# artis-mcrt/artis

Measured on AMD Instinct MI355X. Metric: packet-steps/sec, higher is better.
Workload: dtype f64

## Files before the change

artis_amd/csrc/artis_engine.hip:

```cpp
#include <hip/hip_runtime.h>
#include <rccl/rccl.h>

#include <dlfcn.h>

#include <cstdio>
#include <cstdlib>
#include <algorithm>
#include <chrono>
#include <cstring>
#include <string>
#include <type_traits>
#include <utility>
#include <vector>
#include <cmath>

#include "model_build.h"
#include "engine_config.h"
#include "cache_residency.h"
#include "physics.h"
#include "radfield_fit.h"
#include "ion_balance.h"
#include "decay_update.h"
#include "deposition.h"
#include "spectra.h"
// ... 1050 lines not shown
        Q.s0[s] = w.s0; Q.s1[s] = w.s1; Q.s2[s] = w.s2; Q.s3[s] = w.s3;
        Q.lv[s] = w.ma_level | (k.start << 16);
        Q.cnt[s] = units | (k.njumps << 16);
        Q.ready[nready + __popcll(pm & (lanebit - 1ull))] = (uint8_t)s;
      }
      nready += __popcll(pm);
#ifdef ARTIS_PROFILE
      if (lane == 0) {
        ARTIS_STAT_ADD(env, 46, prof_rounds);
        ARTIS_STAT_ADD(env, 45, prof_lanes);
      }
#endif
      __builtin_amdgcn_wave_barrier();
      TQ_PROF(43);
    }
  }
  __syncthreads();
  if (threadIdx.x < ARTIS_NSTATS && lstats[threadIdx.x] != 0) atomicAdd(&gstats[threadIdx.x], lstats[threadIdx.x]);
}
#ifndef ARTIS_TQ_TB
#define ARTIS_TQ_TB 768
#endif
constexpr int TQ_TB = ARTIS_TQ_TB;
inline size_t tq_lds_bytes(int tb, int nlevels, int nalltrans) {
  return (((sizeof(TQWave) * (size_t)(tb / 64)) + 15) & ~(size_t)15) + (sizeof(LevelPack) * (size_t)nlevels) + (sizeof(uint32_t) * (size_t)((nalltrans + 1) / 2));
}

#ifndef ARTIS_LATE_KERNEL
#define ARTIS_LATE_KERNEL (!ARTIS_OPT_VPKT_ON && !ARTIS_OPT_DETAILED_BF_ESTIMATORS_ON)
#endif
#ifndef ARTIS_LATE_TB
#define ARTIS_LATE_TB 512
#endif
constexpr int LATE_TB = ARTIS_LATE_TB;
constexpr size_t LATE_LDS_HEAD = (sizeof(stat_t) * ARTIS_NSTATS) + 64;
inline size_t late_lds_bytes(int nlevels, int nalltrans, int nbfcontinua) {
  return LATE_LDS_HEAD + (sizeof(LevelPack) * (size_t)nlevels) + (((sizeof(uint32_t) * (size_t)((nalltrans + 1) / 2)) + 15) & ~(size_t)15) +
         (sizeof(ContPack) * (size_t)nbfcontinua);
}
struct LateArgs {
  const int32_t *list[2];
  int32_t n[2];
  int32_t *ring[2];
  int32_t *bailouts;
  int32_t poll_cap;
};
#if ARTIS_LATE_KERNEL
struct LateRing {
  int32_t *ring;
  uint32_t cap;
  int32_t *head, *res, *pub;
};
__device__ inline void late_push(const LateRing &Q, bool flag, int32_t pi, int32_t *errflag) {
  const unsigned long long mask = __ballot(flag);
  if (mask == 0) return;
  const int lane = threadIdx.x & 63;
  const int cnt = __popcll(mask);
  const int prefix = __popcll(mask & ((1ull << lane) - 1ull));
  const int leader = __ffsll((long long)mask) - 1;
  int base = 0;
  if (lane == leader) base = atomicAdd(Q.res, cnt);
  base = __shfl(base, leader);
  if (flag) Q.ring[(uint32_t)(base + prefix) % Q.cap] = pi;
  __builtin_amdgcn_fence(__ATOMIC_RELEASE, "workgroup");
  if (lane == leader) {
    int spins = 0;
    bool turn = true;
    while (__hip_atomic_load(Q.pub, __ATOMIC_RELAXED, __HIP_MEMORY_SCOPE_WORKGROUP) != base) {
      __builtin_amdgcn_s_sleep(1);
      if (++spins > (1 << 24)) {
        if (errflag) *errflag = 47;
        turn = false;
        break;
      }
    }
    if (turn) __hip_atomic_store(Q.pub, base + cnt, __ATOMIC_RELEASE, __HIP_MEMORY_SCOPE_WORKGROUP);
  }
}
__device__ inline int32_t late_pull(const LateRing &Q, bool need) {
  const unsigned long long mask = __ballot(need);
  if (mask == 0) return -1;
  const int lane = threadIdx.x & 63;
  const int prefix = __popcll(mask & ((1ull << lane) - 1ull));
  const int leader = __ffsll((long long)mask) - 1;
  int h = 0, t = 0;
  if (lane == leader) {
    h = __hip_atomic_load(Q.head, __ATOMIC_RELAXED, __HIP_MEMORY_SCOPE_WORKGROUP);
    t = __hip_atomic_load(Q.pub, __ATOMIC_ACQUIRE, __HIP_MEMORY_SCOPE_WORKGROUP);
  }
  h = __shfl(h, leader);
  t = __shfl(t, leader);
  const int take = min(__popcll(mask), t - h);
  if (take <= 0) return -1;
  int32_t v = -1;
  if (need && prefix < take) v = __hip_atomic_load(&Q.ring[(uint32_t)(h + prefix) % Q.cap], __ATOMIC_RELAXED, __HIP_MEMORY_SCOPE_WORKGROUP);
  int ok = 0;
  if (lane == leader) ok = (atomicCAS(Q.head, h, h + take) == h) ? 1 : 0;
  ok = __shfl(ok, leader);
  __builtin_amdgcn_fence(__ATOMIC_ACQUIRE, "workgroup");
  return ok ? v : -1;
}
struct LateSink {
  LateRing q[2];
  int32_t *live;
  int32_t *errflag;
  __device__ void put(bool left, int kind, int32_t pi, const Pkt &p, const Lists &next) const {
    const bool to_r = left && kind == NEXT_RPKT;
    const bool to_t = left && (kind == NEXT_MA || kind == NEXT_KPKT);
    late_push(q[0], to_r, pi, errflag);
    late_push(q[1], to_t, pi, errflag);
    const bool out = left && !to_r && !to_t;
    append_by_kind(out ? kind : NEXT_DONE, pi, p.cellindex, p.nu_cmf, next, (p.ma_element * 5 + p.ma_ion));
    const unsigned long long om = __ballot(out);
    if (om != 0 && (int)(threadIdx.x & 63) == __ffsll((long long)om) - 1) atomicSub(live, __popcll(om));
  }
};
__global__ void __launch_bounds__(LATE_TB, 1) k_late(Env env, LateArgs a, Lists next, unsigned long long *gstats) {
  extern __shared__ __attribute__((aligned(16))) unsigned char late_lds[];
  const int64_t nwg = gridDim.x, b = xcd_chunk(blockIdx.x, nwg);
  const int32_t r0 = (int32_t)(((int64_t)a.n[0] * b) / nwg), r1 = (int32_t)(((int64_t)a.n[0] * (b + 1)) / nwg);
  const int32_t t0 = (int32_t)(((int64_t)a.n[1] * b) / nwg), t1 = (int32_t)(((int64_t)a.n[1] * (b + 1)) / nwg);
  const int32_t own = (r1 - r0) + (t1 - t0);
  if (own == 0) return;
  stat_t *lstats = (stat_t *)late_lds;
  int32_t *ctr = (int32_t *)(late_lds + (sizeof(stat_t) * ARTIS_NSTATS));
  LevelPack *lds_levelpack = (LevelPack *)(late_lds + LATE_LDS_HEAD);
  uint16_t *lds_tlevel = (uint16_t *)(lds_levelpack + env.M.nlevels);
  ContPack *lds_cont = (ContPack *)((unsigned char *)lds_tlevel + (((sizeof(uint32_t) * (size_t)((env.M.nalltrans + 1) / 2)) + 15) & ~(size_t)15));
  if (threadIdx.x < ARTIS_NSTATS) lstats[threadIdx.x] = 0;
  for (int i = threadIdx.x; i < env.M.nlevels; i += LATE_TB) lds_levelpack[i] = env.M.level_pack[i];
  {
    const uint32_t *src = (const uint32_t *)env.M.alltrans_tlevel16;
    uint32_t *dst = (uint32_t *)lds_tlevel;
    for (int i = threadIdx.x; i < (env.M.nalltrans + 1) / 2; i += LATE_TB) dst[i] = src[i];
  }
  {
    const D2 *src = (const D2 *)env.M.cont_pack;
    D2 *dst = (D2 *)lds_cont;
    for (int i = threadIdx.x; i < env.M.nbfcontinua * 2; i += LATE_TB) dst[i] = src[i];
  }
  LateSink sink{{{a.ring[0] + (r0 + t0), (uint32_t)own, ctr + 0, ctr + 2, ctr + 4}, {a.ring[1] + (r0 + t0), (uint32_t)own, ctr + 1, ctr + 3, ctr + 5}},
                ctr + 6, env.errflag};
  for (int i = threadIdx.x; i < r1 - r0; i += LATE_TB) sink.q[0].ring[i] = a.list[0][r0 + i];
  for (int i = threadIdx.x; i < t1 - t0; i += LATE_TB) sink.q[1].ring[i] = a.list[1][t0 + i];
  if (threadIdx.x == 0) {
    ctr[0] = ctr[1] = 0;
    ctr[2] = ctr[4] = r1 - r0;
    ctr[3] = ctr[5] = t1 - t0;
    ctr[6] = own;
  }
  env.M.level_pack = lds_levelpack;
  env.M.alltrans_tlevel16 = lds_tlevel;
  env.ma_tables_in_lds = 1;
  env.M.cont_pack = lds_cont;
  env.cont_in_lds = 1;
  env.cellest_lds = nullptr;
  env.cellest_n = 0;
  env.estcache = nullptr;
  env.estcache_nv = 0;
  __syncthreads();
  env.stats = lstats;
  const double ts_end = env.S.ts_end;
  constexpr int NW = LATE_TB / 64;
  int nw_r = (int)((((int64_t)(r1 - r0) * NW) + (own / 2)) / own);
  if (r1 > r0 && t1 > t0) nw_r = max(1, min(NW - 1, nw_r));
  int role = __builtin_amdgcn_readfirstlane(((int)(threadIdx.x >> 6) < nw_r) ? 0 : 1);
  bool have = false;
  int32_t pi = 0;
  int n_it = 0;
  int polls = 0;
  Pkt p;
  Chi x;
  MACtx k;
  long long tprev = 0;
  while (true) {
    const int32_t got = late_pull(sink.q[role], !have);
    if (got >= 0) {
      pi = got;
      if (role == 0) {
        pkt_load(env.P, pi, p);
        chi_load(env.P, pi, p, x);
      } else {
        pkt_load_thermal(env.P, pi, p);
        k = ma_ctx(env, p);
      }
      have = true;
    }
    if (!__any(have)) {
      const int mine = __hip_atomic_load(ctr + 4 + role, __ATOMIC_RELAXED, __HIP_MEMORY_SCOPE_WORKGROUP) -
                       __hip_atomic_load(ctr + role, __ATOMIC_RELAXED, __HIP_MEMORY_SCOPE_WORKGROUP);
      const int other = __hip_atomic_load(ctr + 5 - role, __ATOMIC_RELAXED, __HIP_MEMORY_SCOPE_WORKGROUP) -
                        __hip_atomic_load(ctr + 1 - role, __ATOMIC_RELAXED, __HIP_MEMORY_SCOPE_WORKGROUP);
      if (__builtin_amdgcn_readfirstlane(mine) > 0) continue;
      if (__builtin_amdgcn_readfirstlane(other) > 0) {
        role = 1 - role;
        continue;
      }
      if (__builtin_amdgcn_readfirstlane(__hip_atomic_load(ctr + 6, __ATOMIC_RELAXED, __HIP_MEMORY_SCOPE_WORKGROUP)) == 0) break;
      if (++polls > a.poll_cap) {
        if ((threadIdx.x & 63) == 0) atomicAdd(a.bailouts, 1);
        break;
      }
      __builtin_amdgcn_s_sleep(64);
      continue;
    }
    polls = 0;
    const bool held = have;
    constexpr bool COLD = false;
#define ROUND_LEAVE(n) false
#define ROUND_BEFORE_LEAVE
#define ROUND_PUT(kind_, pi_) sink.put(held && !have, kind_, pi_, p, next)
    if (role == 0) {
      int &steps = n_it;
#include "rpkt_round.inc"
    } else {
      int &units = n_it;
#include "thermal_round.inc"
    }
#undef ROUND_LEAVE
#undef ROUND_BEFORE_LEAVE
#undef ROUND_PUT
  }
  __syncthreads();
  if (threadIdx.x < ARTIS_NSTATS && lstats[threadIdx.x] != 0) atomicAdd(&gstats[threadIdx.x], lstats[threadIdx.x]);
}
#endif

struct TailLists {
  const int32_t *list[4];
// ... 286 lines not shown
        continue;
      }
      if (have) have = vray_step(env, ray);
    }
  } else {
    for (int64_t i = (int64_t)blockIdx.x * TB + threadIdx.x; i < n64; i += (int64_t)gridDim.x * TB) {
      const VpktSeed seed = queue[i / nobs];
      vpkt_trace_seed_direction(env, seed, (int)(i % nobs));
    }
  }
  __syncthreads();
  if (threadIdx.x < ARTIS_NSTATS && lstats[threadIdx.x] != 0) atomicAdd(&gstats[threadIdx.x], lstats[threadIdx.x]);
}
#endif

inline int nblocks(int64_t n) { return (int)((n + BLOCK - 1) / BLOCK); }

struct SpecState;
void spec_free(SpecState *st);
struct RfState;
void rf_free(RfState *st);
struct IbState;
void ib_free(IbState *st);
struct DecayState;
void decay_free(DecayState *st);
struct DepState;
void dep_free(DepState *st);

}

struct LastCall {
  double propagate_ms = 0., kms[NEXT_NKINDS] = {}, kms_tail = 0., fill_ms = 0.;
  double kms_late = 0.;
  int64_t late_launches = 0;
  int64_t late_bailouts = 0;
  int64_t klaunches[NEXT_NKINDS] = {}, kthreads[NEXT_NKINDS] = {}, nlaunches = 0;
  int64_t sweeps = 0, tile_fills = 0, sparse_fills = 0, cells_filled = 0, listed = 0, parked = 0;
  int64_t pool_resets = 0;
  int32_t thermal_variants = 0, est_forms = 0;
};
struct SortScratch {
  void *base = nullptr;
  int64_t capacity = 0;
  int2 *pairs = nullptr;
  int32_t *mat = nullptr;
  int32_t *tiles = nullptr;
  int32_t *seg = nullptr;
  int32_t *chunk_base = nullptr;
};
struct CellCache {
  int ntiles = 1;
  int tile_lo = 0, tile_hi = 0;
  int tile_valid_lo = -1;
  artis_residency::Residency res;
  int32_t *d_krow = nullptr;
  std::vector<int32_t> h_cell_grid;
  size_t cache_bytes_per_cell = 0;
  int32_t *d_fill_cells = nullptr;
  bool sparse_fill = true;
  int64_t sparse_max_listed = 16384;
  bool tile_adapt = true;
  int64_t tile_block = 0;
  bool pool_keep = true;
  int32_t *d_waiting = nullptr;
  std::vector<int32_t> h_waiting;
  double *d_collexc_terms = nullptr;
  int64_t pop_batch = 0;
// ... 43 lines not shown
  int64_t npackets = -1;
  void *d_pkt = nullptr;
  void *d_pkt_snapshot = nullptr;
  size_t pkt_bytes = 0;
  PktStore P{};
  artis_packet *d_aos = nullptr;
  int64_t aos_capacity = 0;
  bool aos_valid = false;
  int32_t *d_lists[NEXT_NKINDS][2] = {};
  int32_t *d_keys[NEXT_NKINDS][2] = {};
  int32_t *d_sorted = nullptr;
  int32_t *d_perm = nullptr;
  bool use_perm = false;
  bool slot_order_by_cell = true;
  int32_t *d_hist = nullptr;
  int32_t *d_tiles = nullptr;
  SortScratch sort_scratch;
  bool sort_attr_set = false;
  int32_t *d_count = nullptr;
  int32_t *d_cursors = nullptr;
  int ncu = 256;
  double *d_gamma_ws = nullptr;
  int32_t *d_gamma_gi = nullptr;
  int32_t *d_gamma_n = nullptr;
  int64_t ws_capacity = 0;
  hipEvent_t ev0 = nullptr, ev1 = nullptr, ev2 = nullptr, ev3 = nullptr;
  LastCall last;
  int tail_max = ARTIS_OPT_DETAILED_BF_ESTIMATORS_ON ? 16384 : 4096;
  bool tail_always = false;
  int64_t late_max = 200000;
  bool late_always = false;
  bool late_strict = false;
  bool late_attr_set = false;
  int32_t *d_late_ring[2] = {nullptr, nullptr};
  int32_t *d_late_bail = nullptr;
  bool park_tails = true;
  int64_t park_at = 3145728;
  int64_t last_pool_used = 0, last_pool_cap = 0;
  double ma_hotfrac = 1.;
  bool vpkt_cont_lds = true;
  bool tile_zigzag = false;
  int64_t last_visits = 0;
  int budget_r = (ARTIS_OPT_RPKT_BB_THERMALISATION || ARTIS_OPT_VPKT_ON) ? 8 : 4;
  int budget_g = ARTIS_OPT_DETAILED_BF_ESTIMATORS_ON ? 32 : 64;
  int budget_t = ARTIS_OPT_DETAILED_BF_ESTIMATORS_ON ? 1024 : 2048;
  int small_list = 300000;
  int budget_t_small = 0;
  int budget_r_small = 0;
  int drain_t = 48;
  int drain_r = 1;
  int64_t drain_min_list = 1000000;
  bool sort_lists = true;
  bool sort_nu = true;
  bool sort_numajor = true;
  int sort_cellshift = 0;
  bool sort_ma = true;
  bool rpkt_est_over_cont = true;
  int ma_bins = SORT_MABINS;
  bool ma_filters = true;
  int dense_lpr = 32;
  bool dense_cont_lds = true;
  bool cellest_in_lds = true;
  bool estcache = true;
  int sort_maxpc_r = 20000;
  int sort_maxpc_t = 600;
  bool wave_chunks_r = true, wave_chunks_t = false;
  bool cu_chunks_t = false;
  bool cont_lds = true;
// ... 192 lines not shown
  const int32_t matlen = nb * ntiles;
  const int nscan = (matlen + SCAN_TILE - 1) / SCAN_TILE;
  const size_t lds = sizeof(int32_t) * 2 * ((size_t)1 << lobits);
  if (lds > 32 * 1024 && !e->sort_attr_set) {
    HIP_TRY(hipFuncSetAttribute((const void *)k_sort_segments, hipFuncAttributeMaxDynamicSharedMemorySize, (int)(sizeof(int32_t) * 2 << SORT_LO_BITS_MAX)));
    e->sort_attr_set = true;
  }
  hipLaunchKernelGGL(k_sort_tilehist, dim3(ntiles), dim3(SORT_TB), 0, s, keys, n, lobits, nb, ntiles, S.mat);
  hipLaunchKernelGGL(k_scan_tiles, dim3(nscan), dim3(1024), 0, s, S.mat, matlen, S.tiles);
  if (nscan > 1) {
    hipLaunchKernelGGL(k_scan_totals, dim3(1), dim3(1024), 0, s, S.tiles, nscan);
    hipLaunchKernelGGL(k_scan_add, dim3(nscan), dim3(1024), 0, s, S.mat, matlen, S.tiles);
  }
  hipLaunchKernelGGL(k_sort_tilescatter, dim3(ntiles), dim3(SORT_TB), 0, s, list, keys, n, lobits, nb, ntiles, S.mat, S.pairs);
  hipLaunchKernelGGL(k_sort_plan, dim3(1), dim3(1024), 0, s, S.mat, ntiles, nb, n, S.seg, S.chunk_base);
  hipLaunchKernelGGL(k_sort_segments, dim3(n / SORT_SEG_CAP + nb), dim3(BLOCK), lds, s, S.pairs, lobits, nb, S.seg, S.chunk_base, out);
  return ARTIS_OK;
}
int sort_list(artis_amd_engine *e, hipStream_t s, const int32_t *list, const int32_t *keys, int32_t n, int64_t nkeys, int32_t *out) {
  if (nkeys > SORT_LDS_KEYS) return sort_many_keys(e, e->sort_scratch, s, list, keys, n, nkeys, out);
  const int32_t nk = (int32_t)nkeys;
  HIP_TRY(hipMemsetAsync(e->d_hist, 0, sizeof(int32_t) * (size_t)(nk + 1), s));
  hipLaunchKernelGGL(k_sort_hist_lds, dim3(sort_lds_grid(n)), dim3(BLOCK), 0, s, keys, n, e->d_hist, nk);
  const int ntiles = (nk + SCAN_TILE - 1) / SCAN_TILE;
  hipLaunchKernelGGL(k_scan_tiles, dim3(ntiles), dim3(1024), 0, s, e->d_hist, nk, e->d_tiles);
  hipLaunchKernelGGL(k_scan_totals, dim3(1), dim3(1024), 0, s, e->d_tiles, ntiles);
  hipLaunchKernelGGL(k_scan_add, dim3(ntiles), dim3(1024), 0, s, e->d_hist, nk, e->d_tiles);
  hipLaunchKernelGGL(k_sort_scatter_lds, dim3(sort_lds_grid(n)), dim3(BLOCK), 0, s, list, keys, n, e->d_hist, out, nk);
  return ARTIS_OK;
}

void free_packet_buffers(artis_amd_engine *e) {
  void **singles[] = {&e->d_pkt, &e->d_pkt_snapshot, (void **)&e->d_sorted, (void **)&e->d_perm, (void **)&e->d_gamma_ws,
                      (void **)&e->d_late_ring[0], (void **)&e->d_late_ring[1],
                      (void **)&e->d_gamma_gi, (void **)&e->d_gamma_n, (void **)&e->d_bfev, (void **)&e->d_bfev_count,
                      (void **)&e->d_vpkt_queue, (void **)&e->d_vpkt_count};
  e->bfev_cap = 0;
  e->vpkt_cap = 0;
  sort_scratch_free(e->sort_scratch);
  for (void **q : singles) {
    if (*q) (void)hipFree(*q);
    *q = nullptr;
  }
  for (int kind = 0; kind < NEXT_NKINDS; kind++)
    for (int k = 0; k < 2; k++) {
      if (e->d_lists[kind][k]) (void)hipFree(e->d_lists[kind][k]);
      if (e->d_keys[kind][k]) (void)hipFree(e->d_keys[kind][k]);
      e->d_lists[kind][k] = nullptr;
      e->d_keys[kind][k] = nullptr;
    }
  e->npackets = -1;
  e->use_perm = false;
}

bool late_possible(const artis_amd_engine *e) {
  return ARTIS_LATE_KERNEL && e->late_max > 0 && e->tail_max > 0 && e->cc.ntiles == 1 && e->Mh.ncold == 0 && e->Mh.nlevels > 0 && e->Mh.nlevels < 32768 &&
         e->Mh.nalltrans > 0 && e->Mh.nbfcontinua > 0 && late_lds_bytes(e->Mh.nlevels, e->Mh.nalltrans, e->Mh.nbfcontinua) <= 160 * 1024 - 1024;
}
int ensure_packet_buffers(artis_amd_engine *e, int64_t n) {
  if (n == e->npackets && e->d_pkt) return ARTIS_OK;
  free_packet_buffers(e);
  e->pkt_bytes = pkt_store_bytes(n);
  HIP_TRY(hipMalloc(&e->d_pkt, e->pkt_bytes));
  e->P = carve_pkt_store(e->d_pkt, n);
  const size_t listbytes = sizeof(int32_t) * (size_t)(n > 0 ? n : 1);
  for (int kind = 1; kind < NEXT_NKINDS; kind++)
    for (int k = 0; k < 2; k++) {
      HIP_TRY(hipMalloc((void **)&e->d_lists[kind][k], listbytes));
      HIP_TRY(hipMalloc((void **)&e->d_keys[kind][k], listbytes));
    }
  HIP_TRY(hipMalloc((void **)&e->d_sorted, listbytes));
  HIP_TRY(hipMalloc((void **)&e->d_perm, listbytes));
  if (late_possible(e)) {
    for (int k = 0; k < 2; k++) HIP_TRY(hipMalloc((void **)&e->d_late_ring[k], listbytes));
  }
  if (const int rc = sort_scratch_alloc(e->sort_scratch, n)) return rc;
  e->ws_capacity = n > 0 ? n : 1;
  const size_t wsbytes = sizeof(double) * (size_t)(e->Mh.nbfcontinua_ground + 1) * (size_t)e->ws_capacity;
  HIP_TRY(hipMalloc((void **)&e->d_gamma_ws, wsbytes));
  HIP_TRY(hipMalloc((void **)&e->d_gamma_gi, wsbytes / 2));
  HIP_TRY(hipMalloc((void **)&e->d_gamma_n, sizeof(int32_t) * (size_t)e->ws_capacity));
  HIP_TRY(hipMemset(e->d_gamma_n, 0, sizeof(int32_t) * (size_t)e->ws_capacity));
#if ARTIS_OPT_DETAILED_BF_ESTIMATORS_ON
  if (e->Mh.nbfcontinua > 0) {
    const int64_t cap = std::min<int64_t>((int64_t)(n > 0 ? n : 1) * e->budget_r, 0x7FFFFFF0LL);
    HIP_TRY(hipMalloc((void **)&e->d_bfev, sizeof(BfEvent) * (size_t)cap));
    HIP_TRY(hipMalloc((void **)&e->d_bfev_count, sizeof(int32_t)));
    HIP_TRY(hipMemset(e->d_bfev_count, 0, sizeof(int32_t)));
    e->bfev_cap = (int32_t)cap;
  }
#endif
#if ARTIS_OPT_VPKT_ON
  {
    const int64_t cap = std::min<int64_t>((int64_t)(n > 0 ? n : 1) * std::max(e->budget_r, 1), 0x7FFFFFF0LL);
    HIP_TRY(hipMalloc((void **)&e->d_vpkt_queue, sizeof(VpktSeed) * (size_t)cap));
    HIP_TRY(hipMalloc((void **)&e->d_vpkt_count, sizeof(int32_t)));
    HIP_TRY(hipMemset(e->d_vpkt_count, 0, sizeof(int32_t)));
    e->vpkt_cap = (int32_t)cap;
  }
#endif
  e->npackets = n;
  return ARTIS_OK;
}

int ensure_aos(artis_amd_engine *e, int64_t n) {
  if (n <= e->aos_capacity && e->d_aos) return ARTIS_OK;
  if (e->d_aos) (void)hipFree(e->d_aos);
// ... 1032 lines not shown
  if (!e) return ARTIS_ERR_ARG;
  if (sweeps) *sweeps = e->last.sweeps;
  if (tile_fills) *tile_fills = e->last.tile_fills;
  if (fill_ms) *fill_ms = e->last.fill_ms;
  if (listed) *listed = e->last.listed;
  return ARTIS_OK;
}

int artis_amd_last_kernel_table(artis_amd_engine *e, double ms[4], int64_t launches[4], int64_t packets[4]) {
  if (!e) return ARTIS_ERR_ARG;
  const int kinds[4] = {NEXT_RPKT, NEXT_MA, NEXT_KPKT, NEXT_SLOW};
  for (int i = 0; i < 4; i++) {
    if (ms) ms[i] = e->last.kms[kinds[i]];
    if (launches) launches[i] = e->last.klaunches[kinds[i]];
    if (packets) packets[i] = e->last.kthreads[kinds[i]];
  }
  return ARTIS_OK;
}

int artis_amd_last_kernel_ms_by_kind(artis_amd_engine *e, double ms[8], int64_t launches[8]) {
  if (!e || !ms) return ARTIS_ERR_ARG;
  const int kinds[5] = {NEXT_RPKT, NEXT_MA, NEXT_SLOW, NEXT_GAMMA, NEXT_BB};
  for (int i = 0; i < 8; i++) {
    ms[i] = 0.;
    if (launches) launches[i] = 0;
  }
  for (int i = 0; i < 5; i++) {
    ms[i] = e->last.kms[kinds[i]];
    if (launches) launches[i] = e->last.klaunches[kinds[i]];
  }
  ms[5] = e->last.kms_tail;
  ms[6] = e->last.fill_ms;
  ms[7] = e->last.kms_late;
  if (launches) launches[7] = e->last.late_launches;
  return ARTIS_OK;
}

int artis_amd_debug_visit_counts(artis_amd_engine *e, uint32_t *counts, int64_t n) {
  if (!e || !counts || n != (int64_t)e->Mh.npts_nonempty * e->Mh.nlevels) {
    g_last_error = "visit counts: [npts_nonempty][nlevels] uint32 expected";
    return ARTIS_ERR_ARG;
  }
  if (e->d_visit_counts == nullptr) {
    g_last_error = "this library was not built with -DARTIS_VISIT_COUNTS (or no propagation call has run yet)";
    return ARTIS_ERR_ARG;
  }
  HIP_TRY(hipSetDevice(e->device));
  HIP_TRY(hipMemcpy(counts, e->d_visit_counts, sizeof(uint32_t) * (size_t)n, hipMemcpyDeviceToHost));
  return ARTIS_OK;
}

int artis_amd_debug_sort_list(artis_amd_engine *e, const int32_t *keys, const int32_t *list, int32_t n, int64_t nkeys, int32_t *out) {
  if (!e || n < 0 || (n > 0 && (!keys || !list || !out))) {
    g_last_error = "null argument or negative length";
    return ARTIS_ERR_ARG;
  }
  if (nkeys <= SORT_LDS_KEYS) {
    g_last_error = "debug_sort_list runs the many-keys sort: nkeys has to be above " + std::to_string(SORT_LDS_KEYS);
    return ARTIS_ERR_ARG;
  }
  if (nkeys > SORT_MAX_KEYS) {
    g_last_error = sort_too_many_keys_text(nkeys);
    return ARTIS_ERR_UNSUPPORTED;
  }
  for (int32_t i = 0; i < n; i++)
    if (keys[i] < 0 || keys[i] >= nkeys) {
      g_last_error = "a key is outside [0, nkeys)";
// ... 43 lines not shown
```

artis_amd/csrc/stage_propagate.h:

```cpp
#pragma once
namespace {
#define STEP(expr)                     \
  do {                                 \
    const int _rc = (expr);            \
    if (_rc != ARTIS_OK) return _rc;   \
  } while (0)
template <int N>
using Int = std::integral_constant<int, N>;
int sort_by_key(artis_amd_engine *e, hipStream_t s, const int32_t *list, const int32_t *keys, int32_t n, const int32_t **out, int nbins,
                int64_t ncells, int max_per_cell, int32_t nkeys_given = 0, int32_t *into = nullptr) {
  *out = list;
  if (!e->sort_lists || n < 2 * BLOCK) return ARTIS_OK;
  if ((int64_t)n > (int64_t)max_per_cell * (ncells > 0 ? ncells : 1)) return ARTIS_OK;
  if (into == nullptr) into = e->d_sorted;
  STEP(sort_list(e, s, list, keys, n, nkeys_given > 0 ? (int64_t)nkeys_given : (int64_t)e->Mh.ngrid * nbins, into));
  *out = into;
  return ARTIS_OK;
}
#if ARTIS_OPT_DETAILED_BF_ESTIMATORS_ON
void launch_bfest_dense(artis_amd_engine *e, const Env &env, hipStream_t s) {
  const bool lds = e->dense_cont_lds && e->Mh.nbfcontinua <= CONT_LDS_MAX;
  e->last.est_forms |= (lds ? ARTIS_AMD_EST_BF_DENSE_CONTLDS : ARTIS_AMD_EST_BF_DENSE_HBM) |
                       (e->dense_lpr == 64 ? ARTIS_AMD_EST_BF_LPR64 : (e->dense_lpr == 16 ? ARTIS_AMD_EST_BF_LPR16 : ARTIS_AMD_EST_BF_LPR32));
  auto launch = [&](auto lpr) {
// ... 208 lines not shown
      e->last.thermal_variants |= ARTIS_AMD_THERMAL_PLAIN;
      e->last.est_forms |= thermal_est_form(env, 0);
      launch(Int<ARTIS_THERMAL_TB>{}, Int<0>{}, grid, per_cu ? 256 : chunk_count(e->wave_chunks_t, nk, grid * (ARTIS_THERMAL_TB / 64)), per_cu ? 2 : 0);
    }
    return ARTIS_OK;
  }
  void launch_gamma(const int32_t *lst, int32_t nk, const Lists &next) {
    const int grid = std::min(nblocks(nk), e->ncu * ARTIS_GAMMA_WAVES);
    e->last.est_forms |= env.cellest_n_g > 0 ? ARTIS_AMD_EST_GAMMA_LDS : ARTIS_AMD_EST_GAMMA_GLOBAL;
    hipLaunchKernelGGL(k_gamma, dim3(grid), dim3(BLOCK), 0, s, env, lst, nk, next, e->d_stats, e->budget_g, e->d_cursors,
                       chunk_count(e->wave_chunks_r, nk, grid * (BLOCK / 64)));
  }
  int launch_vpkt_followup([[maybe_unused]] int kind) {
#if ARTIS_OPT_VPKT_ON
    if (kind != NEXT_GAMMA && kind != NEXT_BB) {
      HIP_TRY(hipMemsetAsync(e->d_cursors, 0, sizeof(int32_t) * (MAX_CHUNKS + 1), s));
      if (e->vpkt_cont_lds && e->Mh.nbfcontinua <= CONT_LDS_MAX && e->Mh.nbfcontinua > 0)
        hipLaunchKernelGGL((k_vpkt<true, ARTIS_VPKT_TB>), dim3(e->ncu), dim3(ARTIS_VPKT_TB), 0, s, env, e->d_stats, e->d_cursors);
      else
        hipLaunchKernelGGL((k_vpkt<false, BLOCK>), dim3(e->ncu * ARTIS_VPKT_WGS), dim3(BLOCK), 0, s, env, e->d_stats, e->d_cursors);
      HIP_TRY(hipMemsetAsync(e->d_vpkt_count, 0, sizeof(int32_t), s));
    }
#endif
    return ARTIS_OK;
  }
  int finish_launch(int kind, bool tail, int32_t n) {
    HIP_TRY(hipEventRecord(e->ev1, s));
    if (!tail) wall_launch += since(t_launch);
    STEP(read_counts());
    float ms = 0.f;
    HIP_TRY(hipEventElapsedTime(&ms, e->ev0, e->ev1));
    e->last.nlaunches++;
    (tail ? e->last.kms_tail : e->last.kms[kind]) += ms;
    if (!tail) {
      e->last.klaunches[kind]++;
      e->last.kthreads[kind] += n;
      visit_launches++;
    }
    if (e->trace && tail)
      fprintf(stderr, "[artis_amd] launch %lld tail n=%d+0 %.3f ms -> r %d ma %d slow %d gamma %d bb %d\n", (long long)e->last.nlaunches, n, ms, cnt[NEXT_RPKT], cnt[NEXT_MA], cnt[NEXT_NKINDS], cnt[NEXT_GAMMA], cnt[NEXT_BB]);
    else if (e->trace)
      fprintf(stderr, "[artis_amd] launch %lld kind %d n=%d %.3f ms -> r %d ma %d slow %d k %d self %d\n", (long long)e->last.nlaunches, kind, n, ms, cnt[NEXT_RPKT], cnt[NEXT_MA], cnt[NEXT_SLOW], cnt[NEXT_KPKT], cnt[NEXT_NKINDS]);
    cur[kind] = 1 - cur[kind];
    cnt[kind] = cnt[NEXT_NKINDS];
    HIP_TRY(hipMemcpyAsync(e->d_count + kind, e->d_count + NEXT_NKINDS, sizeof(int32_t), hipMemcpyDeviceToDevice, s));
    if (++guard > 2000000LL) {
      g_last_error = "packet loop did not terminate";
      return ARTIS_ERR_NOTCONVERGED;
    }
    return ARTIS_OK;
  }
  static constexpr int tail_kinds[4] = {NEXT_RPKT, NEXT_MA, NEXT_SLOW, NEXT_BB};
  int64_t count_tail() const { return (int64_t)cnt[NEXT_RPKT] + cnt[NEXT_MA] + cnt[NEXT_SLOW] + cnt[NEXT_BB]; }
  int run_tail(int64_t tail_n) {
    TailLists in;
    for (int i = 0; i < 4; i++) {
      in.list[i] = e->d_lists[tail_kinds[i]][cur[tail_kinds[i]]];
      in.n[i] = cnt[tail_kinds[i]];
      HIP_TRY(hipMemsetAsync(e->d_count + tail_kinds[i], 0, sizeof(int32_t), s));
    }
    HIP_TRY(hipMemsetAsync(e->d_count + NEXT_NKINDS, 0, sizeof(int32_t), s));
    STEP(reset_pool_if_due());
    HIP_TRY(hipEventRecord(e->ev0, s));
    e->last.thermal_variants |= ARTIS_AMD_THERMAL_TAIL;
    hipLaunchKernelGGL(k_tail, dim3(nblocks(tail_n * 64)), dim3(BLOCK), 0, s, env, in, lists_for(NEXT_SLOW), e->d_stats);
    STEP(flush_bf_events());
    return finish_launch(NEXT_SLOW, true, (int32_t)tail_n);
  }
  int sort_current(int kind, const int32_t **lst, int32_t *into = nullptr) {
    *lst = e->d_lists[kind][cur[kind]];
    if (kind == NEXT_RPKT || kind == NEXT_GAMMA || (kind == NEXT_MA && e->sort_ma)) {
      STEP(sort_by_key(e, s, e->d_lists[kind][cur[kind]], e->d_keys[kind][cur[kind]], cnt[kind], lst,
                       kind == NEXT_RPKT ? r_nubins : (kind == NEXT_MA ? e->ma_bins : 1), e->cc.res.tile_cells,
                       kind == NEXT_MA ? (env.cellest_n_t > 0 ? INT32_MAX : e->sort_maxpc_t) : (env.cellest_n_r > 0 ? INT32_MAX : e->sort_maxpc_r),
                       (kind == NEXT_RPKT && r_nubins > 1 && e->sort_numajor) ? r_ngroups * r_nubins : 0, into));
    }
    return ARTIS_OK;
  }
  bool late_eligible() const { return late_possible(e) && e->d_late_ring[0] != nullptr; }
  int run_late() {
#if ARTIS_LATE_KERNEL
    LateArgs a;
    const int kinds[2] = {NEXT_RPKT, NEXT_MA};
    const clk::time_point t_sort = clk::now();
    for (int i = 0; i < 2; i++) {
      STEP(sort_current(kinds[i], &a.list[i], e->d_lists[kinds[i]][1 - cur[kinds[i]]]));
      a.n[i] = cnt[kinds[i]];
      a.ring[i] = e->d_late_ring[i];
    }
    wall_sort += since(t_sort);
    a.bailouts = e->d_late_bail;
    a.poll_cap = 1 << 20;
    const size_t lds = late_lds_bytes(e->Mh.nlevels, e->Mh.nalltrans, e->Mh.nbfcontinua);
    if (!e->late_attr_set) {
      HIP_TRY(hipFuncSetAttribute((const void *)k_late, hipFuncAttributeMaxDynamicSharedMemorySize, 160 * 1024 - 1024));
      e->late_attr_set = true;
    }
    for (int i = 0; i < 2; i++) HIP_TRY(hipMemsetAsync(e->d_count + kinds[i], 0, sizeof(int32_t), s));
    HIP_TRY(hipMemsetAsync(e->d_late_bail, 0, sizeof(int32_t), s));
    HIP_TRY(hipEventRecord(e->ev0, s));
    e->last.thermal_variants |= ARTIS_AMD_THERMAL_LATE;
    hipLaunchKernelGGL(k_late, dim3(e->ncu), dim3(LATE_TB), lds, s, env, a, lists_for(0), e->d_stats);
    HIP_TRY(hipEventRecord(e->ev1, s));
    STEP(read_counts());
    const int32_t bail = e->h_counts[(2 * NEXT_NKINDS) + 1];
    float ms = 0.f;
    HIP_TRY(hipEventElapsedTime(&ms, e->ev0, e->ev1));
    e->last.nlaunches++;
    e->last.kms_late += ms;
    e->last.late_launches++;
    e->last.late_bailouts += bail;
    if (e->trace)
      fprintf(stderr, "[artis_amd] launch %lld late n=%d+%d %.3f ms -> slow %d gamma %d bb %d; %d waves gave up waiting\n", (long long)e->last.nlaunches, a.n[0],
              a.n[1], ms, cnt[NEXT_SLOW], cnt[NEXT_GAMMA], cnt[NEXT_BB], bail);
    if (bail != 0 && e->late_strict) {
      g_last_error = "k_late: " + std::to_string(bail) + " waves gave up waiting for work (ARTIS_AMD_LATE_STRICT=1)";
      return ARTIS_ERR_NOTCONVERGED;
    }
    if (++guard > 2000000LL) {
      g_last_error = "packet loop did not terminate";
      return ARTIS_ERR_NOTCONVERGED;
    }
#endif
    return ARTIS_OK;
  }
  int run_kind(int kind) {
    const int32_t nk = cnt[kind];
    const Lists next = lists_for(kind);
    const int32_t *lst = e->d_lists[kind][cur[kind]];
    const clk::time_point t_sort = clk::now();
    STEP(sort_current(kind, &lst));
    wall_sort += since(t_sort);
    t_launch = clk::now();
    if (kind == NEXT_SLOW) STEP(reset_pool_if_due());
    hipLaunchKernelGGL(k_launch_reset, dim3(1), dim3(BLOCK), 0, s, e->d_count, kind, e->d_cursors);
    HIP_TRY(hipEventRecord(e->ev0, s));
    if (kind == NEXT_RPKT)
      STEP(launch_rpkt(lst, nk, next));
    else if (kind == NEXT_GAMMA)
      launch_gamma(lst, nk, next);
    else if (kind == NEXT_MA)
      STEP(launch_thermal(lst, nk, next));
    else if (kind == NEXT_BB)
      hipLaunchKernelGGL(k_blackbody, dim3(nblocks(nk)), dim3(BLOCK), 0, s, env, lst, nk, next, e->d_stats);
    else
      hipLaunchKernelGGL(k_slow, dim3(nblocks(nk)), dim3(BLOCK), 0, s, env, lst, nk, next, e->d_stats);
    STEP(launch_vpkt_followup(kind));
    return finish_launch(kind, false, nk);
  }
  bool should_park(int sweep, int tile, int64_t tail_n, bool tail_now) {
    if (!e->park_tails || e->cc.ntiles <= 1 || visit_launches == 0) return false;
    if (e->park_at > e->tail_max && listed > e->park_at && tail_n > 0 && tail_n + cnt[NEXT_KPKT] <= e->park_at) {
      e->last.parked += tail_n + cnt[NEXT_KPKT] + cnt[NEXT_GAMMA];
      if (e->trace) fprintf(stderr, "[artis_amd] sweep %d tile %d: %lld packets parked (park_at)\n", sweep, tile, (long long)(tail_n + cnt[NEXT_KPKT]));
      return true;
    }
    if (tail_now && listed > e->tail_max) {
      e->last.parked += tail_n + cnt[NEXT_GAMMA];
      if (e->trace) fprintf(stderr, "[artis_amd] sweep %d tile %d: %lld packets parked\n", sweep, tile, (long long)tail_n);
      return true;
    }
    return false;
  }
  int run_visit(int sweep, int tile) {
    static constexpr int order[6] = {NEXT_SLOW, NEXT_GAMMA, NEXT_BB, NEXT_KPKT, NEXT_MA, NEXT_RPKT};
    e->last_visits++;
    listed = count_listed();
    e->last.listed += listed;
    visit_launches = 0;
    if (e->trace) fprintf(stderr, "[artis_amd] sweep %d tile %d of %d\n", sweep, tile, e->cc.ntiles);
    const bool tail_ok = e->tail_max > 0 && (e->tail_always || listed > e->tail_max || sweep > 0 || (adaptive && e->last_visits > e->cc.ntiles));
    const bool late_ok = late_eligible() && (e->late_always || listed > e->late_max);
    while (count_listed() > 0) {
      const int64_t tail_n = count_tail();
      const bool tail_now = tail_ok && tail_n > 0 && tail_n <= e->tail_max && cnt[NEXT_KPKT] == 0;
      if (should_park(sweep, tile, tail_n, tail_now)) break;
      if (tail_now) {
        STEP(run_tail(tail_n));
        continue;
      }
      if (late_ok && cnt[NEXT_KPKT] == 0 && (int64_t)cnt[NEXT_RPKT] + cnt[NEXT_MA] <= e->late_max && cnt[NEXT_BB] <= e->late_max) {
        if (cnt[NEXT_RPKT] + cnt[NEXT_MA] > 0) STEP(run_late());
        for (int kind : order)
          if (kind == NEXT_SLOW || kind == NEXT_GAMMA || kind == NEXT_BB)
            if (cnt[kind] > 0) STEP(run_kind(kind));
        continue;
      }
      for (int kind : order)
        if (cnt[kind] > 0) STEP(run_kind(kind));
    }
    return ARTIS_OK;
  }
};
}
extern "C" int artis_amd_update_packets_device(artis_amd_engine *e, void *hip_stream) {
  if (!e || !e->have_cells || !e->d_pkt) {
    g_last_error = "engine needs artis_amd_set_cellstate() and resident packets first";
    return ARTIS_ERR_ARG;
  }
  HIP_TRY(hipSetDevice(e->device));
  e->fit_since_step = false;
  hipStream_t s = (hipStream_t)hip_stream;
  e->last = {};
  if (e->npackets == 0) return ARTIS_OK;
#ifdef ARTIS_VISIT_COUNTS
  const size_t vb = sizeof(uint32_t) * (size_t)e->Mh.npts_nonempty * (size_t)e->Mh.nlevels;
  if (e->d_visit_counts == nullptr) HIP_TRY(hipMalloc((void **)&e->d_visit_counts, vb));
  HIP_TRY(hipMemsetAsync(e->d_visit_counts, 0, vb, s));
#endif
  PropRun run{e, s};
  if (e->d_bfrate_kept != nullptr) {
    if (e->bfrate_kept_dirty)
      HIP_TRY(hipMemsetAsync(e->d_bfrate_kept, 0, sizeof(double) * (size_t)e->Mh.npts_nonempty * (size_t)e->Mh.nbfcontinua, s));
    e->bfrate_kept_dirty = true;
  }
  const PropRun::clk::time_point wall_t0 = PropRun::clk::now();
  if (e->cc.ntiles > 1 && e->cc.d_waiting == nullptr) {
    HIP_TRY(hipMalloc((void **)&e->cc.d_waiting, sizeof(int32_t) * (size_t)(e->Mh.npts_nonempty + 1)));
// ... 43 lines not shown
```

Measured before the change: 1.446 billion.

## Handle slow packets inside the persistent late kernel via a third work queue

Adds a third ring queue to the persistent k_late kernel so packets routed to the slow path are processed in-kernel by a dedicated wave (with wave-wide free-bound selection) rather than by separate run_kind launches. The late path is now checked before the tail/park logic in the visit loop, and slow packets no longer drop out of the late kernel. This is meant to cut kernel launches and host round trips during the sparse late phase, at the cost of dedicating one wave per workgroup to slow work and more queue contention. Optional profiling counters are compiled in only under ARTIS_PROFILE_LATE.

After: 1.466 billion, median of 6. 1.01x the previous value.

```diff
diff --git a/artis_amd/csrc/artis_engine.hip b/artis_amd/csrc/artis_engine.hip
--- a/artis_amd/csrc/artis_engine.hip
+++ b/artis_amd/csrc/artis_engine.hip
@@ -1106,18 +1106,28 @@
 #ifndef ARTIS_LATE_TB
 #define ARTIS_LATE_TB 512
 #endif
+#ifndef ARTIS_LATE_SLOW_INLINE
+#define ARTIS_LATE_SLOW_INLINE ARTIS_OPT_PHIXS_CLASSIC_NO_INTERPOLATION
+#endif
+#ifndef ARTIS_LATE_SLOW_WAVE
+#define ARTIS_LATE_SLOW_WAVE 1
+#endif
 constexpr int LATE_TB = ARTIS_LATE_TB;
 constexpr size_t LATE_LDS_HEAD = (sizeof(stat_t) * ARTIS_NSTATS) + 64;
 inline size_t late_lds_bytes(int nlevels, int nalltrans, int nbfcontinua) {
   return LATE_LDS_HEAD + (sizeof(LevelPack) * (size_t)nlevels) + (((sizeof(uint32_t) * (size_t)((nalltrans + 1) / 2)) + 15) & ~(size_t)15) +
          (sizeof(ContPack) * (size_t)nbfcontinua);
 }
+constexpr int LATE_NQ = 3;
 struct LateArgs {
-  const int32_t *list[2];
-  int32_t n[2];
-  int32_t *ring[2];
+  const int32_t *list[LATE_NQ];
+  int32_t n[LATE_NQ];
+  int32_t *ring[LATE_NQ];
   int32_t *bailouts;
   int32_t poll_cap;
+#ifdef ARTIS_PROFILE_LATE
+  int32_t *stamp;
+#endif
 };
 #if ARTIS_LATE_KERNEL
 struct LateRing {
@@ -1175,26 +1185,80 @@
   return ok ? v : -1;
 }
 struct LateSink {
-  LateRing q[2];
+  LateRing q[LATE_NQ];
   int32_t *live;
   int32_t *errflag;
+#ifdef ARTIS_PROFILE_LATE
+  int32_t *stamp;
+#endif
   __device__ void put(bool left, int kind, int32_t pi, const Pkt &p, const Lists &next) const {
     const bool to_r = left && kind == NEXT_RPKT;
     const bool to_t = left && (kind == NEXT_MA || kind == NEXT_KPKT);
+    const bool to_s = left && kind == NEXT_SLOW;
+#ifdef ARTIS_PROFILE_LATE
+    if (to_s) stamp[pi] = (int32_t)(clock64() >> 4);
+#endif
     late_push(q[0], to_r, pi, errflag);
     late_push(q[1], to_t, pi, errflag);
-    const bool out = left && !to_r && !to_t;
+    late_push(q[2], to_s, pi, errflag);
+    const bool out = left && !to_r && !to_t && !to_s;
     append_by_kind(out ? kind : NEXT_DONE, pi, p.cellindex, p.nu_cmf, next, (p.ma_element * 5 + p.ma_ion));
     const unsigned long long om = __ballot(out);
     if (om != 0 && (int)(threadIdx.x & 63) == __ffsll((long long)om) - 1) atomicSub(live, __popcll(om));
   }
 };
+#if ARTIS_LATE_SLOW_INLINE
+__device__ inline
+#else
+__device__ __noinline__
+#endif
+void late_slow_round(const Env &env, const LateSink &sink, const Lists &next, int32_t got) {
+  const bool mine = got >= 0;
+  const int32_t pi = mine ? got : 0;
+  Pkt p;
+  p.cellindex = 0; p.nu_cmf = 0.; p.ma_element = 0; p.ma_ion = 0;
+  FbSel sel;
+  sel.mode = 1;
+  sel.valid = false;
+  sel.element = sel.lowerion = sel.lower = sel.t = 0;
+  sel.T_e = 0.f;
+  sel.zrand = sel.nu = 0.;
+  if (mine) pkt_load(env.P, pi, p);
+#ifdef ARTIS_PROFILE_LATE
+  const long long tpass0 = clock64();
+  if (mine) {
+    const uint32_t w = (uint32_t)((int32_t)(tpass0 >> 4) - sink.stamp[pi]);
+    atomicAdd(&env.stats[42], (stat_t)w);
+    atomicAdd(&env.stats[43], (stat_t)1);
+    if (w > (1u << 12)) atomicAdd(&env.stats[44], (stat_t)1);
+    if (w > (1u << 16)) atomicAdd(&env.stats[45], (stat_t)1);
+  }
+#endif
+  if (mine && slow_selects_continuum_nu(p)) {
+    Pkt t = p;
+    (void)advance_slow(env, t, pi, &sel);
+  }
+  fbsel_wave(env, sel);
+  int kind = NEXT_DONE;
+  if (mine) {
+    kind = advance_slow(env, p, pi, sel.valid ? &sel : nullptr);
+    pkt_store(env.P, pi, p);
+  }
+  sink.put(mine, kind, pi, p, next);
+#ifdef ARTIS_PROFILE_LATE
+  if ((threadIdx.x & 63) == 0) {
+    atomicAdd(&env.stats[46], (stat_t)1);
+    atomicAdd(&env.stats[47], (stat_t)((clock64() - tpass0) >> 4));
+  }
+#endif
+}
 __global__ void __launch_bounds__(LATE_TB, 1) k_late(Env env, LateArgs a, Lists next, unsigned long long *gstats) {
   extern __shared__ __attribute__((aligned(16))) unsigned char late_lds[];
   const int64_t nwg = gridDim.x, b = xcd_chunk(blockIdx.x, nwg);
   const int32_t r0 = (int32_t)(((int64_t)a.n[0] * b) / nwg), r1 = (int32_t)(((int64_t)a.n[0] * (b + 1)) / nwg);
   const int32_t t0 = (int32_t)(((int64_t)a.n[1] * b) / nwg), t1 = (int32_t)(((int64_t)a.n[1] * (b + 1)) / nwg);
-  const int32_t own = (r1 - r0) + (t1 - t0);
+  const int32_t s0 = (int32_t)(((int64_t)a.n[2] * b) / nwg), s1 = (int32_t)(((int64_t)a.n[2] * (b + 1)) / nwg);
+  const int32_t own = (r1 - r0) + (t1 - t0) + (s1 - s0);
   if (own == 0) return;
   stat_t *lstats = (stat_t *)late_lds;
   int32_t *ctr = (int32_t *)(late_lds + (sizeof(stat_t) * ARTIS_NSTATS));
@@ -1213,14 +1277,27 @@
     D2 *dst = (D2 *)lds_cont;
     for (int i = threadIdx.x; i < env.M.nbfcontinua * 2; i += LATE_TB) dst[i] = src[i];
   }
-  LateSink sink{{{a.ring[0] + (r0 + t0), (uint32_t)own, ctr + 0, ctr + 2, ctr + 4}, {a.ring[1] + (r0 + t0), (uint32_t)own, ctr + 1, ctr + 3, ctr + 5}},
-                ctr + 6, env.errflag};
+  const int32_t slice = r0 + t0 + s0;
+  LateSink sink{{{a.ring[0] + slice, (uint32_t)own, ctr + 0, ctr + 2, ctr + 4}, {a.ring[1] + slice, (uint32_t)own, ctr + 1, ctr + 3, ctr + 5},
+                 {a.ring[2] + slice, (uint32_t)own, ctr + 7, ctr + 8, ctr + 9}},
+                ctr + 6, env.errflag
+#ifdef ARTIS_PROFILE_LATE
+                , a.stamp
+#endif
+  };
   for (int i = threadIdx.x; i < r1 - r0; i += LATE_TB) sink.q[0].ring[i] = a.list[0][r0 + i];
   for (int i = threadIdx.x; i < t1 - t0; i += LATE_TB) sink.q[1].ring[i] = a.list[1][t0 + i];
+  for (int i = threadIdx.x; i < s1 - s0; i += LATE_TB) {
+    sink.q[2].ring[i] = a.list[2][s0 + i];
+#ifdef ARTIS_PROFILE_LATE
+    a.stamp[a.list[2][s0 + i]] = (int32_t)(clock64() >> 4);
+#endif
+  }
   if (threadIdx.x == 0) {
-    ctr[0] = ctr[1] = 0;
+    ctr[0] = ctr[1] = ctr[7] = 0;
     ctr[2] = ctr[4] = r1 - r0;
     ctr[3] = ctr[5] = t1 - t0;
+    ctr[8] = ctr[9] = s1 - s0;
     ctr[6] = own;
   }
   env.M.level_pack = lds_levelpack;
@@ -1236,9 +1313,17 @@
   env.stats = lstats;
   const double ts_end = env.S.ts_end;
   constexpr int NW = LATE_TB / 64;
-  int nw_r = (int)((((int64_t)(r1 - r0) * NW) + (own / 2)) / own);
-  if (r1 > r0 && t1 > t0) nw_r = max(1, min(NW - 1, nw_r));
-  int role = __builtin_amdgcn_readfirstlane(((int)(threadIdx.x >> 6) < nw_r) ? 0 : 1);
+  constexpr int NW_RT = ARTIS_LATE_SLOW_WAVE ? NW - 1 : NW;
+  const int32_t own_rt = (r1 - r0) + (t1 - t0);
+  int nw_r = own_rt > 0 ? (int)((((int64_t)(r1 - r0) * NW_RT) + (own_rt / 2)) / own_rt) : 0;
+  if (r1 > r0 && t1 > t0) nw_r = max(1, min(NW_RT - 1, nw_r));
+  const bool slow_wave = ARTIS_LATE_SLOW_WAVE && __builtin_amdgcn_readfirstlane((int)(threadIdx.x >> 6)) == NW - 1;
+  int home = __builtin_amdgcn_readfirstlane(((int)(threadIdx.x >> 6) < nw_r) ? 0 : 1);
+  int role = slow_wave ? 2 : home;
+  const auto waiting = [&](int q) {
+    return __builtin_amdgcn_readfirstlane(__hip_atomic_load(sink.q[q].pub, __ATOMIC_RELAXED, __HIP_MEMORY_SCOPE_WORKGROUP) -
+                                          __hip_atomic_load(sink.q[q].head, __ATOMIC_RELAXED, __HIP_MEMORY_SCOPE_WORKGROUP));
+  };
   bool have = false;
   int32_t pi = 0;
   int n_it = 0;
@@ -1249,7 +1334,13 @@
   long long tprev = 0;
   while (true) {
     const int32_t got = late_pull(sink.q[role], !have);
-    if (got >= 0) {
+    if (role == 2) {
+      if (__any(got >= 0)) {
+        late_slow_round(env, sink, next, got);
+        polls = 0;
+        continue;
+      }
+    } else if (got >= 0) {
       pi = got;
       if (role == 0) {
         pkt_load(env.P, pi, p);
@@ -1261,14 +1352,17 @@
       have = true;
     }
     if (!__any(have)) {
-      const int mine = __hip_atomic_load(ctr + 4 + role, __ATOMIC_RELAXED, __HIP_MEMORY_SCOPE_WORKGROUP) -
-                       __hip_atomic_load(ctr + role, __ATOMIC_RELAXED, __HIP_MEMORY_SCOPE_WORKGROUP);
-      const int other = __hip_atomic_load(ctr + 5 - role, __ATOMIC_RELAXED, __HIP_MEMORY_SCOPE_WORKGROUP) -
-                        __hip_atomic_load(ctr + 1 - role, __ATOMIC_RELAXED, __HIP_MEMORY_SCOPE_WORKGROUP);
-      if (__builtin_amdgcn_readfirstlane(mine) > 0) continue;
-      if (__builtin_amdgcn_readfirstlane(other) > 0) {
-        role = 1 - role;
+      if (waiting(2) > 0) {
+        role = 2;
         continue;
+      }
+      if (!slow_wave) {
+        role = home;
+        if (waiting(home) > 0) continue;
+        if (waiting(1 - home) > 0) {
+          role = home = 1 - home;
+          continue;
+        }
       }
       if (__builtin_amdgcn_readfirstlane(__hip_atomic_load(ctr + 6, __ATOMIC_RELAXED, __HIP_MEMORY_SCOPE_WORKGROUP)) == 0) break;
       if (++polls > a.poll_cap) {
@@ -1621,7 +1715,7 @@
 struct LastCall {
   double propagate_ms = 0., kms[NEXT_NKINDS] = {}, kms_tail = 0., fill_ms = 0.;
   double kms_late = 0.;
-  int64_t late_launches = 0;
+  int64_t late_launches = 0, tail_launches = 0;
   int64_t late_bailouts = 0;
   int64_t klaunches[NEXT_NKINDS] = {}, kthreads[NEXT_NKINDS] = {}, nlaunches = 0;
   int64_t sweeps = 0, tile_fills = 0, sparse_fills = 0, cells_filled = 0, listed = 0, parked = 0;
@@ -1731,8 +1825,11 @@
   bool late_always = false;
   bool late_strict = false;
   bool late_attr_set = false;
-  int32_t *d_late_ring[2] = {nullptr, nullptr};
+  int32_t *d_late_ring[LATE_NQ] = {nullptr, nullptr, nullptr};
   int32_t *d_late_bail = nullptr;
+#ifdef ARTIS_PROFILE_LATE
+  int32_t *d_late_stamp = nullptr;
+#endif
   bool park_tails = true;
   int64_t park_at = 3145728;
   int64_t last_pool_used = 0, last_pool_cap = 0;
@@ -1991,7 +2088,7 @@
 
 void free_packet_buffers(artis_amd_engine *e) {
   void **singles[] = {&e->d_pkt, &e->d_pkt_snapshot, (void **)&e->d_sorted, (void **)&e->d_perm, (void **)&e->d_gamma_ws,
-                      (void **)&e->d_late_ring[0], (void **)&e->d_late_ring[1],
+                      (void **)&e->d_late_ring[0], (void **)&e->d_late_ring[1], (void **)&e->d_late_ring[2],
                       (void **)&e->d_gamma_gi, (void **)&e->d_gamma_n, (void **)&e->d_bfev, (void **)&e->d_bfev_count,
                       (void **)&e->d_vpkt_queue, (void **)&e->d_vpkt_count};
   e->bfev_cap = 0;
@@ -2031,7 +2128,7 @@
   HIP_TRY(hipMalloc((void **)&e->d_sorted, listbytes));
   HIP_TRY(hipMalloc((void **)&e->d_perm, listbytes));
   if (late_possible(e)) {
-    for (int k = 0; k < 2; k++) HIP_TRY(hipMalloc((void **)&e->d_late_ring[k], listbytes));
+    for (int k = 0; k < LATE_NQ; k++) HIP_TRY(hipMalloc((void **)&e->d_late_ring[k], listbytes));
   }
   if (const int rc = sort_scratch_alloc(e->sort_scratch, n)) return rc;
   e->ws_capacity = n > 0 ? n : 1;
@@ -3130,7 +3227,10 @@
   ms[5] = e->last.kms_tail;
   ms[6] = e->last.fill_ms;
   ms[7] = e->last.kms_late;
-  if (launches) launches[7] = e->last.late_launches;
+  if (launches) {
+    launches[5] = e->last.tail_launches;
+    launches[7] = e->last.late_launches;
+  }
   return ARTIS_OK;
 }
 
diff --git a/artis_amd/csrc/stage_propagate.h b/artis_amd/csrc/stage_propagate.h
--- a/artis_amd/csrc/stage_propagate.h
+++ b/artis_amd/csrc/stage_propagate.h
@@ -264,6 +264,7 @@
     HIP_TRY(hipEventElapsedTime(&ms, e->ev0, e->ev1));
     e->last.nlaunches++;
     (tail ? e->last.kms_tail : e->last.kms[kind]) += ms;
+    if (tail) e->last.tail_launches++;
     if (!tail) {
       e->last.klaunches[kind]++;
       e->last.kthreads[kind] += n;
@@ -313,14 +314,18 @@
   int run_late() {
 #if ARTIS_LATE_KERNEL
     LateArgs a;
-    const int kinds[2] = {NEXT_RPKT, NEXT_MA};
+    const int kinds[LATE_NQ] = {NEXT_RPKT, NEXT_MA, NEXT_SLOW};
     const clk::time_point t_sort = clk::now();
-    for (int i = 0; i < 2; i++) {
+    for (int i = 0; i < LATE_NQ; i++) {
       STEP(sort_current(kinds[i], &a.list[i], e->d_lists[kinds[i]][1 - cur[kinds[i]]]));
       a.n[i] = cnt[kinds[i]];
       a.ring[i] = e->d_late_ring[i];
     }
     wall_sort += since(t_sort);
+#ifdef ARTIS_PROFILE_LATE
+    if (e->d_late_stamp == nullptr) HIP_TRY(hipMalloc((void **)&e->d_late_stamp, sizeof(int32_t) * (size_t)std::max<int64_t>(e->npackets, 1)));
+    a.stamp = e->d_late_stamp;
+#endif
     a.bailouts = e->d_late_bail;
     a.poll_cap = 1 << 20;
     const size_t lds = late_lds_bytes(e->Mh.nlevels, e->Mh.nalltrans, e->Mh.nbfcontinua);
@@ -328,7 +333,7 @@
       HIP_TRY(hipFuncSetAttribute((const void *)k_late, hipFuncAttributeMaxDynamicSharedMemorySize, 160 * 1024 - 1024));
       e->late_attr_set = true;
     }
-    for (int i = 0; i < 2; i++) HIP_TRY(hipMemsetAsync(e->d_count + kinds[i], 0, sizeof(int32_t), s));
+    for (int i = 0; i < LATE_NQ; i++) HIP_TRY(hipMemsetAsync(e->d_count + kinds[i], 0, sizeof(int32_t), s));
     HIP_TRY(hipMemsetAsync(e->d_late_bail, 0, sizeof(int32_t), s));
     HIP_TRY(hipEventRecord(e->ev0, s));
     e->last.thermal_variants |= ARTIS_AMD_THERMAL_LATE;
@@ -343,8 +348,8 @@
     e->last.late_launches++;
     e->last.late_bailouts += bail;
     if (e->trace)
-      fprintf(stderr, "[artis_amd] launch %lld late n=%d+%d %.3f ms -> slow %d gamma %d bb %d; %d waves gave up waiting\n", (long long)e->last.nlaunches, a.n[0],
-              a.n[1], ms, cnt[NEXT_SLOW], cnt[NEXT_GAMMA], cnt[NEXT_BB], bail);
+      fprintf(stderr, "[artis_amd] launch %lld late n=%d+%d+%d %.3f ms -> slow %d gamma %d bb %d; %d waves gave up waiting\n", (long long)e->last.nlaunches,
+              a.n[0], a.n[1], a.n[2], ms, cnt[NEXT_SLOW], cnt[NEXT_GAMMA], cnt[NEXT_BB], bail);
     if (bail != 0 && e->late_strict) {
       g_last_error = "k_late: " + std::to_string(bail) + " waves gave up waiting for work (ARTIS_AMD_LATE_STRICT=1)";
       return ARTIS_ERR_NOTCONVERGED;
@@ -404,18 +409,18 @@
     const bool tail_ok = e->tail_max > 0 && (e->tail_always || listed > e->tail_max || sweep > 0 || (adaptive && e->last_visits > e->cc.ntiles));
     const bool late_ok = late_eligible() && (e->late_always || listed > e->late_max);
     while (count_listed() > 0) {
+      if (late_ok && cnt[NEXT_KPKT] == 0 && (int64_t)cnt[NEXT_RPKT] + cnt[NEXT_MA] <= e->late_max && cnt[NEXT_BB] <= e->late_max) {
+        if (cnt[NEXT_RPKT] + cnt[NEXT_MA] + cnt[NEXT_SLOW] > 0) STEP(run_late());
+        for (int kind : order)
+          if (kind == NEXT_GAMMA || kind == NEXT_BB)
+            if (cnt[kind] > 0) STEP(run_kind(kind));
+        continue;
+      }
       const int64_t tail_n = count_tail();
       const bool tail_now = tail_ok && tail_n > 0 && tail_n <= e->tail_max && cnt[NEXT_KPKT] == 0;
       if (should_park(sweep, tile, tail_n, tail_now)) break;
       if (tail_now) {
         STEP(run_tail(tail_n));
-        continue;
-      }
-      if (late_ok && cnt[NEXT_KPKT] == 0 && (int64_t)cnt[NEXT_RPKT] + cnt[NEXT_MA] <= e->late_max && cnt[NEXT_BB] <= e->late_max) {
-        if (cnt[NEXT_RPKT] + cnt[NEXT_MA] > 0) STEP(run_late());
-        for (int kind : order)
-          if (kind == NEXT_SLOW || kind == NEXT_GAMMA || kind == NEXT_BB)
-            if (cnt[kind] > 0) STEP(run_kind(kind));
         continue;
       }
       for (int kind : order)
```
